# Yasas1994/Jaeger

Measured on AMD Instinct MI355X. Metric: Mbp/s classified (1500bp frags), higher is better.
Workload: dtype f16x3 (split-f16, f32 accumulate)

## Files before the change

### jaeger_amd/csrc/jg_conv_f16_impl.h

```cpp
#include <stdio.h>
#include <stdlib.h>
#include <type_traits>

#include "jg_common.h"

#include "jg_conv_dev.h"

namespace {


#ifdef JG_STAMP
static __device__ unsigned long long jg_stamp_acc[8];
#define JG_ST_DECL unsigned long long st_[8] = {0, 0, 0, 0, 0, 0, 0, 0}; unsigned long long st_t = __builtin_amdgcn_s_memtime(); const unsigned long long st_t0 = st_t
#define JG_ST(idx) do { const unsigned long long n_ = __builtin_amdgcn_s_memtime(); st_[idx] += n_ - st_t; st_t = n_; } while (0)
#define JG_ST_END do { st_[5] = __builtin_amdgcn_s_memtime() - st_t0; if (lane == 0) { for (int q_ = 0; q_ < 8; ++q_) atomicAdd(&jg_stamp_acc[q_], st_[q_]); } } while (0)
#else
#define JG_ST_DECL
#define JG_ST(idx)
#define JG_ST_END
#endif

#ifndef JG_PRIO
#define JG_PRIO 1
#endif
// ... 555 lines not shown
      }
      ++xc;
    }
    JG_ST(3);

    if (a.dbg & 1) {
      if (acc[0][0][0] + acc[1][TN - 1][3] + acc[TM - 1][TN - 1][7] + acc[TM - 1][0][9] == 12345.678f) a.overflow[0] = 2;
    } else if constexpr (JG_FASTEP && TANH && !LUT && CW == 128 && EP != JG_EP_GENERIC && K == 5) {
      JG_PRIO_EPI();
      constexpr bool HAS_ADD = (EP & JG_EP_ADD) != 0;
      constexpr bool HAS_NMD = (EP & (JG_EP_NMD1 | JG_EP_NMD2)) != 0;
      constexpr int N1 = (EP >> 1) & 3, N2 = (EP >> 6) & 3;
      static_assert(N1 != 2 && N2 != 2, "the tanh-GELU builds carry no DyT stage");
      typedef unsigned u32x4 __attribute__((ext_vector_type(4)));
      const Tile &tile = cur[0];
      float vmax = 0.f;
      bool vnan = false;
      const unsigned L4 = 4u * (unsigned)a.L_out;
      unsigned ob[4], om[4], olive = 0;
#pragma unroll
      for (int tm = 0; tm < 4; ++tm) {
        int row, p;
        const bool live = resolve(tile, (wm * 4 + tm) * 32 + i, a.L_out, row, p);
        const int mc = live ? p : 0;
        if constexpr (FLAT) {
          if (!live) row = min(max(row, 0), a.rows - 1);
        }
        ob[tm] = (unsigned)(((row * 8 + 4 * wn) * 4 + h) * a.L_out + mc);
        om[tm] = (unsigned)(row * a.L_out + mc);
        if (live) olive |= 1u << tm;
      }
      struct In {
        u32x4 sh0, sh1, sl0, sl1;
        unsigned char mkb;
      };
      auto fetch = [&](In &q, int b) {
        const int tm = b & 3, tn = b >> 2;
        q.mkb = a.mask_out != nullptr ? a.mask_out[om[tm]] : (unsigned char)1;
        if constexpr (HAS_ADD) {
          if (!(a.dbg & 128)) {
            const unsigned it0 = ob[tm] + (unsigned)(2 * tn) * L4, it1 = it0 + L4;
            q.sh0 = ld_stream(reinterpret_cast<const u32x4 *>(a.addh + it0));
            q.sl0 = ld_stream(reinterpret_cast<const u32x4 *>(a.addh + it0 + 2u * (unsigned)a.L_out));
            q.sh1 = ld_stream(reinterpret_cast<const u32x4 *>(a.addh + it1));
            q.sl1 = ld_stream(reinterpret_cast<const u32x4 *>(a.addh + it1 + 2u * (unsigned)a.L_out));
          } else {
            q.sh0 = q.sh1 = q.sl0 = q.sl1 = u32x4{0u, 0u, 0u, 0u};
          }
        }
      };
      auto swap32 = [](unsigned &lo_half_keeps, unsigned &hi_half_keeps) {
        const auto r = __builtin_amdgcn_permlane32_swap(lo_half_keeps, hi_half_keeps, false, false);
        lo_half_keeps = r[0];
        hi_half_keeps = r[1];
      };
#define JG_DPP(v, ctrl) __uint_as_float((unsigned)__builtin_amdgcn_update_dpp(0, (int)__float_as_uint(v), (ctrl), 0xf, 0xf, false))
      auto lane_reduce = [&](const float (&in)[16], auto op) -> float {
        const bool b2 = (i & 4) != 0, b1 = (i & 2) != 0, b0 = (i & 1) != 0, b3 = (i & 8) != 0;
        float s8[8], s4[4], s2[2];
#pragma unroll
        for (int q = 0; q < 8; ++q) {
          const float keep = b2 ? in[8 + q] : in[q], send = b2 ? in[q] : in[8 + q];
          s8[q] = op(keep, JG_DPP(send, 0x141));
        }
#pragma unroll
        for (int q = 0; q < 4; ++q) {
          const float keep = b1 ? s8[4 + q] : s8[q], send = b1 ? s8[q] : s8[4 + q];
          s4[q] = op(keep, JG_DPP(send, 0x4e));
        }
#pragma unroll
        for (int q = 0; q < 2; ++q) {
          const float keep = b0 ? s4[2 + q] : s4[q], send = b0 ? s4[q] : s4[2 + q];
          s2[q] = op(keep, JG_DPP(send, 0xb1));
        }
        const float keep1 = b3 ? s2[1] : s2[0], send1 = b3 ? s2[0] : s2[1];
        const float v = op(keep1, JG_DPP(send1, 0x128));
        return op(v, __shfl_xor(v, 16, 32));
      };
#undef JG_DPP
      auto reduced_slot = [&](int tn, int &ch) -> size_t {
        const int r = 8 * (int)((i & 4) != 0) + 4 * (int)((i & 2) != 0) + 2 * (int)((i & 1) != 0) + (int)((i & 8) != 0);
        ch = (wn * 2 + tn) * 32 + 8 * (r >> 2) + 4 * h + (r & 3);
        return ((size_t)tile.T * STRIPS + wm) * a.cout + ch;
      };
      f32x2 nmd2[8];
      float pool_acc[16];
      In in0, in1;
      fetch(in0, 0);
      fetch(in1, 1);
      auto do_block = [&](int b, In &q) {
        const int tm = b & 3, tn = b >> 2;
        f32x16 &x = acc[tm][tn];
        const bool live = ((olive >> tm) & 1u) != 0u;
        const float mk = (live && q.mkb != 0) ? 1.f : 0.f;
        const int nb = (wn * 2 + tn) * 32;
        if (tm == 0) {
          if constexpr (HAS_NMD) {
#pragma unroll
            for (int r = 0; r < 8; ++r) nmd2[r] = f32x2{0.f, 0.f};
          }
#pragma unroll
          for (int r = 0; r < 16; ++r) pool_acc[r] = -INFINITY;
        }
        if (!(a.dbg & 32)) {
#pragma unroll
          for (int j = 0; j < 2; ++j) {
            f32x2 v[4];
#pragma unroll
            for (int r = 0; r < 4; ++r) v[r] = f32x2{x[8 * j + 2 * r], x[8 * j + 2 * r + 1]};
            auto st_affine = [&](int row) {
              const float *pr = epiL + (row * 2) * HN + nb + 4 * h + 16 * j;
              const float4 sc0 = *reinterpret_cast<const float4 *>(pr), sc1 = *reinterpret_cast<const float4 *>(pr + 8);
              const float4 of0 = *reinterpret_cast<const float4 *>(pr + HN), of1 = *reinterpret_cast<const float4 *>(pr + HN + 8);
              v[0] = __builtin_elementwise_fma(v[0], f32x2{sc0.x, sc0.y}, f32x2{of0.x, of0.y});
              v[1] = __builtin_elementwise_fma(v[1], f32x2{sc0.z, sc0.w}, f32x2{of0.z, of0.w});
              v[2] = __builtin_elementwise_fma(v[2], f32x2{sc1.x, sc1.y}, f32x2{of1.x, of1.y});
              v[3] = __builtin_elementwise_fma(v[3], f32x2{sc1.z, sc1.w}, f32x2{of1.z, of1.w});
            };
            auto st_add = [&]() {
              const u32x4 qh = j == 0 ? q.sh0 : q.sh1, ql = j == 0 ? q.sl0 : q.sl1;
              unsigned hx = qh[0], hy = qh[1], hz = qh[2], hw_ = qh[3];
              unsigned lx = ql[0], ly = ql[1], lz = ql[2], lw_ = ql[3];
              swap32(hx, hz); swap32(hy, hw_);
              swap32(lx, lz); swap32(ly, lw_);
              v[0] += f32x2{mix_sum<0>(hx, lx), mix_sum<1>(hx, lx)};
              v[1] += f32x2{mix_sum<0>(hy, ly), mix_sum<1>(hy, ly)};
              v[2] += f32x2{mix_sum<0>(hz, lz), mix_sum<1>(hz, lz)};
              v[3] += f32x2{mix_sum<0>(hw_, lw_), mix_sum<1>(hw_, lw_)};
            };
            auto st_gelu = [&]() {
#pragma unroll
              for (int r = 0; r < 4; ++r) v[r] = fast_gelu2(v[r]);
            };
            auto st_nmd = [&]() {
              const f32x2 mk2 = {mk, mk};
#pragma unroll
              for (int r = 0; r < 4; ++r) nmd2[4 * j + r] = __builtin_elementwise_fma(v[r], mk2, nmd2[4 * j + r]);
            };
            st_affine(0);
            if constexpr (EP & JG_EP_NMD1) st_nmd();
            if constexpr (N1 == 1) st_affine(1);
            if constexpr (HAS_ADD) st_add();
            if constexpr (EP & JG_EP_ACT1) st_gelu();
            if constexpr (EP & JG_EP_NMD2) st_nmd();
            if constexpr (N2 == 1) st_affine(N1 ? 2 : 1);
            if constexpr (EP & JG_EP_ACT2) st_gelu();
            if (a.out_f16s) {
              unsigned hp[4], lp[4];
#pragma unroll
              for (int r = 0; r < 4; ++r) {
                typedef _Float16 half2_t __attribute__((ext_vector_type(2)));
                const half2_t hh = {(_Float16)v[r].x, (_Float16)v[r].y};
                hp[r] = *reinterpret_cast<const unsigned *>(&hh);
                const half2_t ll = {(_Float16)mix_rem<0>(v[r].x, hp[r]), (_Float16)mix_rem<1>(v[r].y, hp[r])};
                lp[r] = *reinterpret_cast<const unsigned *>(&ll);
              }
              vmax = fmaxf(fmaxf(vmax, fmaxf(fabsf(v[0].x), fabsf(v[0].y))), fmaxf(fabsf(v[1].x), fabsf(v[1].y)));
              vmax = fmaxf(fmaxf(vmax, fmaxf(fabsf(v[2].x), fabsf(v[2].y))), fmaxf(fabsf(v[3].x), fabsf(v[3].y)));
              vnan = vnan || __builtin_isunordered(v[0].x, v[0].y) || __builtin_isunordered(v[1].x, v[1].y) ||
                     __builtin_isunordered(v[2].x, v[2].y) || __builtin_isunordered(v[3].x, v[3].y);
              swap32(hp[0], hp[2]); swap32(hp[1], hp[3]);
              swap32(lp[0], lp[2]); swap32(lp[1], lp[3]);
              if (live && !(a.dbg & 64)) {
                uint4 *yh = reinterpret_cast<uint4 *>(a.y);
                const unsigned it4 = ob[tm] + (unsigned)(2 * tn + j) * L4;
                const u32x4 vhi = {hp[0], hp[1], hp[2], hp[3]}, vlo = {lp[0], lp[1], lp[2], lp[3]};
                st_stream(vhi, reinterpret_cast<u32x4 *>(yh + it4));
                st_stream(vlo, reinterpret_cast<u32x4 *>(yh + it4 + 2u * (unsigned)a.L_out));
              }
            } else if (a.pool_out != nullptr) {
#pragma unroll
              for (int r = 0; r < 4; ++r) {
                pool_acc[8 * j + 2 * r] = mk != 0.f ? fmaxf(pool_acc[8 * j + 2 * r], v[r].x) : pool_acc[8 * j + 2 * r];
                pool_acc[8 * j + 2 * r + 1] = mk != 0.f ? fmaxf(pool_acc[8 * j + 2 * r + 1], v[r].y) : pool_acc[8 * j + 2 * r + 1];
              }
            } else if (live && !(a.dbg & 64)) {
              float *yf = reinterpret_cast<float *>(a.y) + (size_t)om[tm] * a.cout + nb + 4 * h + 16 * j;
              *reinterpret_cast<float4 *>(yf) = make_float4(v[0].x, v[0].y, v[1].x, v[1].y);
              *reinterpret_cast<float4 *>(yf + 8) = make_float4(v[2].x, v[2].y, v[3].x, v[3].y);
            }
          }
        }
        if (b + 2 < 8) fetch(q, b + 2);
        if (tm == 3) {
          if constexpr (HAS_NMD) {
            float na[16];
#pragma unroll
            for (int r = 0; r < 8; ++r) { na[2 * r] = nmd2[r].x; na[2 * r + 1] = nmd2[r].y; }
            const float rv = lane_reduce(na, [](float x_, float y_) { return x_ + y_; });
            int ch;
            const size_t slot = reduced_slot(tn, ch);
            if (i < 16 && tile.valid) a.nmd_out[slot] = rv;
          }
          if (a.pool_out != nullptr) {
            const float rv = lane_reduce(pool_acc, [](float x_, float y_) { return fmaxf(x_, y_); });
            int ch;
            const size_t slot = reduced_slot(tn, ch);
            if (i < 16 && tile.valid) a.pool_out[slot] = rv;
          }
        }
      };
#pragma unroll
      for (int bp = 0; bp < 4; ++bp) {
        do_block(2 * bp, in0);
        do_block(2 * bp + 1, in1);
      }
      if ((!(vmax <= 65000.0f) || vnan) && a.overflow != nullptr && a.dbg == 0) atomicOr(a.overflow, 1);
      JG_PRIO_MAIN();
    } else {
      JG_PRIO_EPI();
      float vmax = 0.f;
      bool vnan = false;
      float nmd_acc[16];
      float nmd_acc2[16];
      struct Pre {
        uint2 sh[4], sl[4];
        unsigned char mkb;
      };
      auto swap32 = [](unsigned &lo_half_keeps, unsigned &hi_half_keeps) {
        const auto r = __builtin_amdgcn_permlane32_swap(lo_half_keeps, hi_half_keeps, false, false);
        lo_half_keeps = r[0];
        hi_half_keeps = r[1];
      };
      auto item4 = [&](int row, int mc, int nb, int j) -> unsigned {
        const int G = ((nb + ch0) >> 3) + 2 * j + h;
        return (unsigned)(((row * (a.cout_pad >> 4) + (G >> 1)) * 4 + (G & 1)) * a.L_out + mc);
      };
      const bool psplit = GEN && a.psplit != 0;
      const int L_st = psplit ? ((a.L_out + 1) >> 1) : a.L_out;
      auto item4_out = [&](int row, int mc, int nb, int j) -> unsigned {
        if constexpr (GEN) {
          if (psplit) {
            const int G = ((nb + ch0) >> 3) + 2 * j + h, CC = a.cout_pad >> 4;
            return (unsigned)(((row * 2 * CC + (mc & 1) * CC + (G >> 1)) * 4 + (G & 1)) * L_st + (mc >> 1));
          }
        }
        return item4(row, mc, nb, j);
      };
      auto out_pos = [&](const Tile &tile, int tm, int &row, int &mc) -> bool {
        int p;
        bool live = resolve(tile, (wm * TM + tm) * 32 + i, L_res, row, p);
        if constexpr (GEN) {
          if (a.ostride == 2) {
            live = live && !(p & 1);
            p >>= 1;
          }
        }
        mc = live ? p : 0;
        if constexpr (FLAT) {
          if (!live) row = min(max(row, 0), a.rows - 1);
        }
        return live;
      };
      constexpr bool OPOS = !GEN;
      unsigned ob[TM], om[TM], olive = 0;
      size_t o_row = 0, o_mrow = 0;
      unsigned o_step = 0;
      const void *e_y = a.y, *e_addh = a.addh;
      const uint8_t *e_mask = a.mask_out;
      int e_dbg = a.dbg, e_f16s = a.out_f16s;
      float *e_pool = a.pool_out, *e_nmd = a.nmd_out;
      int *e_overflow = a.overflow;
      if constexpr (OPOS) {
        typedef const __attribute__((address_space(4))) ConvHArgs *KArgs;
        KArgs ka = (KArgs)__builtin_amdgcn_kernarg_segment_ptr();
        asm volatile("" : "+s"(ka));
        e_addh = ka->addh;
        e_mask = ka->mask_out;
        e_dbg = ka->dbg;
        e_f16s = ka->out_f16s;
        e_nmd = ka->nmd_out;
        const unsigned Lo = (unsigned)ka->L_out, CC4 = (unsigned)(ka->cout_pad >> 4) * 4u;
        o_step = FLAT ? 2u * Lo : 32u * Lo;
        asm volatile("" : "+s"(o_step));
        if constexpr (!FLAT) {
          o_row = (size_t)cur[0].rowblk * CC4 * Lo * 16u + (size_t)(wn * 8) * o_step;
          o_mrow = (size_t)cur[0].rowblk * Lo;
        }
#pragma unroll
        for (int tm = 0; tm < TM; ++tm) {
          int row, p;
          const bool live = resolve(cur[0], (wm * TM + tm) * 32 + i, (int)Lo, row, p);
          const int mc = live ? p : 0;
          if constexpr (FLAT) {
            if (!live) row = min(max(row, 0), a.rows - 1);
          }
          if (live) olive |= 1u << tm;
          if constexpr (FLAT) {
            om[tm] = (unsigned)row * Lo + (unsigned)mc;
            ob[tm] = ((unsigned)row * CC4 + (unsigned)h) * Lo + (unsigned)mc;
          } else {
            om[tm] = (unsigned)mc;
            ob[tm] = ((unsigned)h * Lo + (unsigned)mc) * 16u;
          }
        }
      }
      auto o_item = [&](const void *base, int tm, int tn, int j, int plane) -> const char * {
        if constexpr (FLAT) {
          return reinterpret_cast<const char *>(base) + ((size_t)(ob[tm] + (unsigned)(((wn * 2 + tn) * 2 + j) * 2 + plane) * o_step) << 4);
        } else {
          return reinterpret_cast<const char *>(base) + (o_row + (size_t)((unsigned)((tn * 2 + j) * 2 + plane) * o_step)) + ob[tm];
        }
      };
      auto o_maskbyte = [&](int tm) -> unsigned char {
        return e_mask != nullptr ? (e_mask + o_mrow)[om[tm]] : (unsigned char)1;
      };
      auto prefetch = [&](Pre &p, const Tile &tile, int tm, int tn) {
        const int nb = (wn * 2 + tn) * 32;
        int orow = 0, mc = 0;
        if constexpr (OPOS) {
          p.mkb = o_maskbyte(tm);
        } else {
          out_pos(tile, tm, orow, mc);
          p.mkb = a.mask_out != nullptr ? a.mask_out[(size_t)orow * a.L_out + mc] : (unsigned char)1;
        }
        if (e_addh != nullptr && !(e_dbg & 128)) {
#pragma unroll
          for (int j = 0; j < 2; ++j) {
            typedef unsigned u32x4 __attribute__((ext_vector_type(4)));
            const u32x4 *src_h, *src_l;
            if constexpr (OPOS) {
              src_h = reinterpret_cast<const u32x4 *>(o_item(e_addh, tm, tn, j, 0));
              src_l = reinterpret_cast<const u32x4 *>(o_item(e_addh, tm, tn, j, 1));
            } else {
              const unsigned it4 = item4(orow, mc, (!GEN || nb + ch0 + 16 * j < a.cout) ? nb : 0, j);
              src_h = reinterpret_cast<const u32x4 *>(a.addh + it4);
              src_l = reinterpret_cast<const u32x4 *>(a.addh + it4 + 2u * (unsigned)a.L_out);
            }
            const u32x4 nh = ld_stream(src_h);
            const u32x4 nl = ld_stream(src_l);
            uint4 vh = make_uint4(nh[0], nh[1], nh[2], nh[3]);
            uint4 vl = make_uint4(nl[0], nl[1], nl[2], nl[3]);
            swap32(vh.x, vh.z); swap32(vh.y, vh.w);
            swap32(vl.x, vl.z); swap32(vl.y, vl.w);
            p.sh[2 * j] = make_uint2(vh.x, vh.y);  p.sh[2 * j + 1] = make_uint2(vh.z, vh.w);
            p.sl[2 * j] = make_uint2(vl.x, vl.y);  p.sl[2 * j + 1] = make_uint2(vl.z, vl.w);
          }
        } else {
#pragma unroll
          for (int g = 0; g < 4; ++g) p.sh[g] = p.sl[g] = make_uint2(0u, 0u);
        }
      };
      auto epi_block = [&](f32x16 &x, const Tile &tile, int tm, int tn) {
        Pre p;
        prefetch(p, tile, tm, tn);
        const int nb = (wn * 2 + tn) * 32;
        bool live;
        if constexpr (OPOS) {
          live = ((olive >> tm) & 1u) != 0u;
        } else {
          int orow_, mc_;
          live = out_pos(tile, tm, orow_, mc_);
        }
        const float mk = p.mkb != 0 ? 1.f : 0.f;
        auto st_affine = [&](int row) {
          const float *pr = epiL + (row * 2) * HN + nb + 4 * h;
#pragma unroll
          for (int g = 0; g < 4; ++g) {
            const float4 sc = *reinterpret_cast<const float4 *>(pr + 8 * g);
            const float4 of = *reinterpret_cast<const float4 *>(pr + HN + 8 * g);
            x[4 * g + 0] = fmaf(x[4 * g + 0], sc.x, of.x);
            x[4 * g + 1] = fmaf(x[4 * g + 1], sc.y, of.y);
            x[4 * g + 2] = fmaf(x[4 * g + 2], sc.z, of.z);
            x[4 * g + 3] = fmaf(x[4 * g + 3], sc.w, of.w);
          }
        };
        auto st_dyt = [&](int row, float alpha, int use_mask) {
          const float *pr = epiL + (row * 2) * HN + nb + 4 * h;
          const float mm = use_mask ? mk : 1.0f;
#pragma unroll
          for (int g = 0; g < 4; ++g) {
            const float4 ga = *reinterpret_cast<const float4 *>(pr + 8 * g);
            const float4 be = *reinterpret_cast<const float4 *>(pr + HN + 8 * g);
            x[4 * g + 0] = (fast_tanh(alpha * x[4 * g + 0]) * ga.x + be.x) * mm;
            x[4 * g + 1] = (fast_tanh(alpha * x[4 * g + 1]) * ga.y + be.y) * mm;
            x[4 * g + 2] = (fast_tanh(alpha * x[4 * g + 2]) * ga.z + be.z) * mm;
            x[4 * g + 3] = (fast_tanh(alpha * x[4 * g + 3]) * ga.w + be.w) * mm;
          }
        };
        auto st_add = [&]() {
#pragma unroll
          for (int g = 0; g < 4; ++g) {
            x[4 * g + 0] += mix_sum<0>(p.sh[g].x, p.sl[g].x);
            x[4 * g + 1] += mix_sum<1>(p.sh[g].x, p.sl[g].x);
            x[4 * g + 2] += mix_sum<0>(p.sh[g].y, p.sl[g].y);
            x[4 * g + 3] += mix_sum<1>(p.sh[g].y, p.sl[g].y);
          }
        };
        auto st_gelu = [&]() {
          constexpr bool TANH_ONLY = TANH || EP == JG_EP_RUNTIME ||
                                     (EP != JG_EP_GENERIC && ((((EP >> 1) & 3) == 2) || (((EP >> 6) & 3) == 2)));
          if (TANH_ONLY || a.act_kind == JG_ACT_GELU_TANH) {
#pragma unroll
            for (int r = 0; r < 16; ++r) x[r] = fast_gelu(x[r]);
          } else if (a.act_kind == JG_ACT_GELU_ERF) {
#pragma unroll
            for (int r = 0; r < 16; ++r) x[r] = gelu_erf(x[r]);
          } else {
#pragma unroll
            for (int r = 0; r < 16; ++r) x[r] = fmaxf(x[r], 0.0f);
          }
        };
        auto st_nmd = [&](int which = 0) {
          const float mkl = live ? mk : 0.f;
          if constexpr (EP == JG_EP_RUNTIME) {
            if (which) {
#pragma unroll
              for (int r = 0; r < 16; ++r) nmd_acc2[r] = fmaf(x[r], mkl, nmd_acc2[r]);
              return;
            }
          }
#pragma unroll
          for (int r = 0; r < 16; ++r) nmd_acc[r] = fmaf(x[r], mkl, nmd_acc[r]);
        };
        if constexpr (EP == JG_EP_GENERIC) {
          for (int q = 0; q < ((e_dbg & 32) ? 0 : a.n_hst); ++q) {
            const HStageArg st = a.hst[q];
            switch (st.kind) {
              case JG_HST_AFFINE: st_affine(st.pad_); break;
              case JG_HST_DYT: st_dyt(st.pad_, st.f0, st.arg); break;
              case JG_HST_ADD: st_add(); break;
              case JG_HST_ACT:
#pragma unroll
                for (int r = 0; r < 16; ++r) x[r] = jg_act(x[r], st.arg);
                break;
              case JG_HST_NMD: st_nmd(); break;
              case JG_HST_MASKMUL:
#pragma unroll
                for (int r = 0; r < 16; ++r) x[r] *= mk;
                break;
              default: break;
            }
          }
        } else if constexpr (EP == JG_EP_RUNTIME) {
          const unsigned e_ = a.ep_rt;
          const int n1 = (int)((e_ >> 1) & 3u), n2 = (int)((e_ >> 6) & 3u);
          st_affine(0);
          if (e_ & JG_EP_NMD1) st_nmd(0);
          if (n1 == 1) st_affine(1);
          else if (n1 == 2) st_dyt(1, a.alpha1, a.dytmask1);
          if (e_ & JG_EP_ADD) st_add();
          if (e_ & JG_EP_ACT1) st_gelu();
          if (e_ & JG_EP_NMD2) st_nmd((e_ & JG_EP_NMD1) ? 1 : 0);
          if (n2 == 1) st_affine(n1 ? 2 : 1);
          else if (n2 == 2) st_dyt(n1 ? 2 : 1, a.alpha2, a.dytmask2);
          if (e_ & JG_EP_ACT2) st_gelu();
        } else if (!(e_dbg & 32)) {
          constexpr int N1 = (EP >> 1) & 3, N2 = (EP >> 6) & 3;
          st_affine(0);
          if constexpr (EP & JG_EP_NMD1) st_nmd();
          if constexpr (N1 == 1) st_affine(1);
          if constexpr (N1 == 2) st_dyt(1, a.alpha1, a.dytmask1);
          if constexpr (EP & JG_EP_ADD) st_add();
          if constexpr (EP & JG_EP_ACT1) st_gelu();
          if constexpr (EP & JG_EP_NMD2) st_nmd();
          if constexpr (N2 == 1) st_affine(N1 ? 2 : 1);
          if constexpr (N2 == 2) st_dyt(N1 ? 2 : 1, a.alpha2, a.dytmask2);
          if constexpr (EP & JG_EP_ACT2) st_gelu();
        }
        if constexpr (GEN) {
          if (psplit) {
#pragma unroll
            for (int r = 0; r < 16; ++r) x[r] *= mk;
          }
        }
        if (e_f16s) {
          uint2 ph[4], pl[4];
#pragma unroll
          for (int g = 0; g < 4; ++g) {
            half4 hh4, ll4;
#pragma unroll
            for (int j = 0; j < 4; ++j) {
              hh4[j] = (_Float16)x[4 * g + j];
              vmax = fmaxf(vmax, fabsf(x[4 * g + j]));
            }
            vnan = vnan || __builtin_isunordered(x[4 * g + 0], x[4 * g + 1]) || __builtin_isunordered(x[4 * g + 2], x[4 * g + 3]);
            ph[g] = *reinterpret_cast<uint2 *>(&hh4);
            ll4[0] = (_Float16)mix_rem<0>(x[4 * g + 0], ph[g].x);
            ll4[1] = (_Float16)mix_rem<1>(x[4 * g + 1], ph[g].x);
            ll4[2] = (_Float16)mix_rem<0>(x[4 * g + 2], ph[g].y);
            ll4[3] = (_Float16)mix_rem<1>(x[4 * g + 3], ph[g].y);
            pl[g] = *reinterpret_cast<uint2 *>(&ll4);
          }
#pragma unroll
          for (int j = 0; j < 2; ++j) {
            unsigned h0 = ph[2 * j].x, h1 = ph[2 * j].y, h2 = ph[2 * j + 1].x, h3 = ph[2 * j + 1].y;
            unsigned l0 = pl[2 * j].x, l1 = pl[2 * j].y, l2 = pl[2 * j + 1].x, l3 = pl[2 * j + 1].y;
            swap32(h0, h2); swap32(h1, h3);
            swap32(l0, l2); swap32(l1, l3);
            x[4 * j + 0] = __uint_as_float(h0); x[4 * j + 1] = __uint_as_float(h1);
            x[4 * j + 2] = __uint_as_float(h2); x[4 * j + 3] = __uint_as_float(h3);
            x[8 + 4 * j + 0] = __uint_as_float(l0); x[8 + 4 * j + 1] = __uint_as_float(l1);
            x[8 + 4 * j + 2] = __uint_as_float(l2); x[8 + 4 * j + 3] = __uint_as_float(l3);
          }
        }
      };
      char *f32_base = nullptr;
      auto store_block = [&](const f32x16 &x, const Tile &tile, int tm, int tn, bool f16s) {
        const int nb = (wn * 2 + tn) * 32;
        if constexpr (OPOS) {
          typedef unsigned u32x4 __attribute__((ext_vector_type(4)));
          if (f16s) {
#pragma unroll
            for (int j = 0; j < 2; ++j) {
              const u32x4 vhi = {__float_as_uint(x[4 * j]), __float_as_uint(x[4 * j + 1]),
                                 __float_as_uint(x[4 * j + 2]), __float_as_uint(x[4 * j + 3])};
              const u32x4 vlo = {__float_as_uint(x[8 + 4 * j]), __float_as_uint(x[8 + 4 * j + 1]),
                                 __float_as_uint(x[8 + 4 * j + 2]), __float_as_uint(x[8 + 4 * j + 3])};
              st_stream(vhi, reinterpret_cast<u32x4 *>(const_cast<char *>(o_item(e_y, tm, tn, j, 0))));
              st_stream(vlo, reinterpret_cast<u32x4 *>(const_cast<char *>(o_item(e_y, tm, tn, j, 1))));
            }
          } else {
            char *yf = f32_base + tn * (32 * 4);
            if constexpr (FLAT) yf += ((size_t)om[tm] * (HN * 4) + 16 * h);
            else yf += om[tm] * (unsigned)(HN * 4) + 16u * (unsigned)h;
#pragma unroll
            for (int g = 0; g < 4; ++g)
              *reinterpret_cast<float4 *>(yf + 32 * g) = make_float4(x[4 * g], x[4 * g + 1], x[4 * g + 2], x[4 * g + 3]);
          }
          return;
        }
        int orow, mc;
        const bool live = out_pos(tile, tm, orow, mc);
        if (live && !(e_dbg & 64)) {
          if (e_f16s) {
            uint4 *yh = reinterpret_cast<uint4 *>(a.y);
#pragma unroll
            for (int j = 0; j < 2; ++j) {
              if (GEN && nb + ch0 + 16 * j >= a.cout) continue;
              const unsigned it4 = item4_out(orow, mc, nb, j);
              typedef unsigned u32x4 __attribute__((ext_vector_type(4)));
              const u32x4 vhi = {__float_as_uint(x[4 * j]), __float_as_uint(x[4 * j + 1]),
                                 __float_as_uint(x[4 * j + 2]), __float_as_uint(x[4 * j + 3])};
              const u32x4 vlo = {__float_as_uint(x[8 + 4 * j]), __float_as_uint(x[8 + 4 * j + 1]),
                                 __float_as_uint(x[8 + 4 * j + 2]), __float_as_uint(x[8 + 4 * j + 3])};
              st_stream(vhi, reinterpret_cast<u32x4 *>(yh + it4));
              st_stream(vlo, reinterpret_cast<u32x4 *>(yh + it4 + 2u * (unsigned)L_st));
              if (GEN && psplit && (a.L_out & 1) && mc == a.L_out - 1) {
                const unsigned itz = it4 + (unsigned)((a.cout_pad >> 4) * 4 * L_st);
                const u32x4 z = {0u, 0u, 0u, 0u};
                st_stream(z, reinterpret_cast<u32x4 *>(yh + itz));
                st_stream(z, reinterpret_cast<u32x4 *>(yh + itz + 2u * (unsigned)L_st));
              }
            }
          } else {
            float *yf = reinterpret_cast<float *>(a.y) + ((size_t)orow * a.L_out + mc) * a.cout + ch0 + nb + 4 * h;
#pragma unroll
            for (int g = 0; g < 4; ++g)
              if (ch0 + nb + 8 * g + 4 * h < a.cout)
                *reinterpret_cast<float4 *>(yf + 8 * g) =
                    make_float4(x[4 * g], x[4 * g + 1], x[4 * g + 2], x[4 * g + 3]);
          }
        }
      };
#define JG_DPP(v, ctrl) __uint_as_float((unsigned)__builtin_amdgcn_update_dpp(0, (int)__float_as_uint(v), (ctrl), 0xf, 0xf, false))
      auto lane_reduce = [&](const float (&in)[16], auto op) -> float {
        const bool b2 = (i & 4) != 0, b1 = (i & 2) != 0, b0 = (i & 1) != 0, b3 = (i & 8) != 0;
        float s8[8], s4[4], s2[2];
#pragma unroll
        for (int q = 0; q < 8; ++q) {
          const float keep = b2 ? in[8 + q] : in[q], send = b2 ? in[q] : in[8 + q];
          s8[q] = op(keep, JG_DPP(send, 0x141));
        }
#pragma unroll
        for (int q = 0; q < 4; ++q) {
          const float keep = b1 ? s8[4 + q] : s8[q], send = b1 ? s8[q] : s8[4 + q];
          s4[q] = op(keep, JG_DPP(send, 0x4e));
        }
#pragma unroll
        for (int q = 0; q < 2; ++q) {
          const float keep = b0 ? s4[2 + q] : s4[q], send = b0 ? s4[q] : s4[2 + q];
          s2[q] = op(keep, JG_DPP(send, 0xb1));
        }
        const float keep1 = b3 ? s2[1] : s2[0], send1 = b3 ? s2[0] : s2[1];
        const float v = op(keep1, JG_DPP(send1, 0x128));
        return op(v, __shfl_xor(v, 16, 32));
      };
      auto reduced_slot = [&](const Tile &tile, int tn, int &ch) -> size_t {
        const int r = 8 * (int)((i & 4) != 0) + 4 * (int)((i & 2) != 0) + 2 * (int)((i & 1) != 0) + (int)((i & 8) != 0);
        ch = ch0 + (wn * 2 + tn) * 32 + 8 * (r >> 2) + 4 * h + (r & 3);
        return ((size_t)tile.T * STRIPS + wm) * a.cout + ch;
      };
      auto nmd_flush = [&](const Tile &tile, int tn) {
        const float v = lane_reduce(nmd_acc, [](float x, float y) { return x + y; });
        int ch;
        const size_t slot = reduced_slot(tile, tn, ch);
        if (i < 16 && tile.valid && ch < a.cout) e_nmd[slot] = v;
      };
      const bool has_nmd = (EP == JG_EP_GENERIC || EP == JG_EP_RUNTIME) ? e_nmd != nullptr : (EP & (JG_EP_NMD1 | JG_EP_NMD2)) != 0;
#pragma unroll
      for (int tn = 0; tn < TN; ++tn) {
#pragma unroll
        for (int r = 0; r < 16; ++r) nmd_acc[r] = 0.f;
        if constexpr (EP == JG_EP_RUNTIME) {
#pragma unroll
          for (int r = 0; r < 16; ++r) nmd_acc2[r] = 0.f;
        }
#pragma unroll
        for (int tm = 0; tm < TM; ++tm) epi_block(acc[tm][tn], cur[0], tm, tn);
        if (has_nmd) nmd_flush(cur[0], tn);
        if constexpr (EP == JG_EP_RUNTIME) {
          if (a.nmd_out2 != nullptr) {
            const float v2 = lane_reduce(nmd_acc2, [](float x, float y) { return x + y; });
            int ch2;
            const size_t slot2 = reduced_slot(cur[0], tn, ch2);
            if (i < 16 && cur[0].valid && ch2 < a.cout) a.nmd_out2[slot2] = v2;
          }
        }
      }
      if constexpr (OPOS) {
        typedef const __attribute__((address_space(4))) ConvHArgs *KArgs;
        KArgs ka = (KArgs)__builtin_amdgcn_kernarg_segment_ptr();
        asm volatile("" : "+s"(ka));
        e_y = ka->y;
        e_pool = ka->pool_out;
        e_overflow = ka->overflow;
      }
      if (e_pool != nullptr) {
        float mkv[TM];
#pragma unroll
        for (int tm = 0; tm < TM; ++tm) {
          bool live;
          unsigned char mb;
          if constexpr (OPOS) {
            live = ((olive >> tm) & 1u) != 0u;
            mb = o_maskbyte(tm);
          } else {
            int orow, mc;
            live = out_pos(cur[0], tm, orow, mc);
            mb = a.mask_out != nullptr ? a.mask_out[(size_t)orow * a.L_out + mc] : (unsigned char)1;
          }
          mkv[tm] = (live && mb != 0) ? 1.f : 0.f;
        }
#pragma unroll
        for (int tn = 0; tn < TN; ++tn) {
          float pa[16];
#pragma unroll
          for (int r = 0; r < 16; ++r) pa[r] = -INFINITY;
#pragma unroll
          for (int tm = 0; tm < TM; ++tm)
#pragma unroll
            for (int r = 0; r < 16; ++r) pa[r] = mkv[tm] != 0.f ? fmaxf(pa[r], acc[tm][tn][r]) : pa[r];
          const float v = lane_reduce(pa, [](float x, float y) { return fmaxf(x, y); });
          int ch;
          const size_t slot = reduced_slot(cur[0], tn, ch);
          if (i < 16 && cur[0].valid && ch < a.cout) e_pool[slot] = v;
        }
      } else if constexpr (OPOS) {
        auto store_tile = [&](bool f16s) {
#pragma unroll
          for (int tm = 0; tm < TM; ++tm) {
            if (!((olive >> tm) & 1u)) continue;
#pragma unroll
            for (int tn = 0; tn < TN; ++tn) store_block(acc[tm][tn], cur[0], tm, tn, f16s);
          }
        };
        if (!(e_dbg & 64)) {
          if (e_f16s) {
            store_tile(true);
          } else {
            f32_base = reinterpret_cast<char *>(const_cast<void *>(e_y)) + (o_mrow * (size_t)HN + (size_t)(wn * 64)) * 4u;
            store_tile(false);
          }
        }
      } else {
#pragma unroll
        for (int tm = 0; tm < TM; ++tm) {
#pragma unroll
          for (int tn = 0; tn < TN; ++tn) store_block(acc[tm][tn], cur[0], tm, tn, false);
        }
      }
      if ((!(vmax <= 65000.0f) || vnan) && e_overflow != nullptr && e_dbg == 0) atomicOr(e_overflow, 1);
      JG_PRIO_MAIN();
    }
    if constexpr (!PIPE) zero_acc();
#pragma unroll
    for (int u = 0; u < NT; ++u) cur[u] = np[u];
    tiles_of(pass + 2, np);
    if constexpr (!LUT) load_bytes(np);
    JG_ST(4);
  }
#ifdef JG_VALU_PROBE
  if (probe[0] + probe[1] + probe[2] + probe[3] + probe[4] + probe[5] + probe[6] + probe[7] == 12345.678f) a.overflow[0] = 4;
#endif
  JG_ST_END;
}

template <int K, unsigned EP, bool FLAT = false, int CW = 128, bool TANH = false, bool PIPE = false>
int launch_ke(jg_engine *e, const ConvHArgs &a, hipStream_t s) {
  const int smem = jg_conv_f16_lds_bytes(K, a.dil);
  static bool attr_set = false;
  if (!attr_set) {
    JG_HIP(hipFuncSetAttribute(reinterpret_cast<const void *>(conv_f16x3_kernel<K, EP, false, FLAT, CW, TANH, PIPE>),
                               hipFuncAttributeMaxDynamicSharedMemorySize, 160 * 1024));
    attr_set = true;
  }
  const int n_tiles = FLAT ? a.flat_tiles : a.rows * a.tiles_m;
  const int n_pairs = (n_tiles + NT - 1) / NT;
  static const bool one_wg = jg_exp_env("JG_ONE_WG") != nullptr;
  int grid = ((smem <= 80 * 1024 && !one_wg) ? 2 : 1) * e->n_cu;
  if (grid > n_pairs) grid = n_pairs;
  ConvHArgs b = a;
  hipLaunchKernelGGL((conv_f16x3_kernel<K, EP, false, FLAT, CW, TANH, PIPE>), dim3((unsigned)grid), dim3(HT), (size_t)smem, s, b);
  JG_HIP(hipGetLastError());
#ifdef JG_STAMP
  {
    unsigned long long h[8], z[8] = {0, 0, 0, 0, 0, 0, 0, 0};
    JG_HIP(hipStreamSynchronize(s));
    JG_HIP(hipMemcpyFromSymbol(h, HIP_SYMBOL(jg_stamp_acc), sizeof(h)));
    JG_HIP(hipMemcpyToSymbol(HIP_SYMBOL(jg_stamp_acc), z, sizeof(z)));
    const double tot = (double)h[5];
    fprintf(stderr, "STAMP k=%d ep=%u rows=%d grid=%d total_cyc/wave=%.0f wait=%.3f barrier=%.3f issue=%.3f lds_mfma=%.3f epilogue=%.3f\n",
            K, EP, a.rows, grid, tot / (grid * 4.0), h[0] / tot, h[1] / tot, h[2] / tot, (h[3] + h[6]) / tot, h[4] / tot);
  }
#endif
  return JG_OK;
}

template <int K, unsigned EP, bool FLAT>
int launch_hot(jg_engine *e, const ConvHArgs &a, hipStream_t s) {
  if constexpr (K == 5) {
#ifdef JG_EXPERIMENT
    if (e->conv_pc == 2 && a.dil == 3 && a.cc_in % 2 == 0 && a.dbg == 0) return launch_ke<5, EP, FLAT, 128, true, true>(e, a, s);
#endif
    return launch_ke<5, EP, FLAT, 128, true>(e, a, s);
  } else {
    return launch_ke<K, EP, FLAT>(e, a, s);
  }
}

#if JG_CONV_PART == 4
template <unsigned EP, int CW, bool TANH = false>
int launch_lut_e(jg_engine *e, const ConvHArgs &a, hipStream_t s) {
  const int smem = jg_conv_lut_lds_bytes(a.k, a.lut_vocab);
  static bool attr_set = false;
  if (!attr_set) {
    JG_HIP(hipFuncSetAttribute(reinterpret_cast<const void *>(conv_f16x3_kernel<0, EP, true, false, CW, TANH>),
                               hipFuncAttributeMaxDynamicSharedMemorySize, 160 * 1024));
    attr_set = true;
  }
  const int n_tiles = a.rows * a.tiles_m;
  constexpr int tper = JG_LUT_WAVES / 2;
  const int n_pairs = (n_tiles + tper - 1) / tper;
  const int grid = a.lut_one_half ? (n_pairs < e->n_cu ? n_pairs : e->n_cu)
                                  : 2 * (n_pairs < e->n_cu / 2 ? n_pairs : e->n_cu / 2);
  hipLaunchKernelGGL((conv_f16x3_kernel<0, EP, true, false, CW, TANH>), dim3((unsigned)grid), dim3(JG_LUT_WAVES * 64), (size_t)smem, s, a);
  JG_HIP(hipGetLastError());
  return JG_OK;
}

int launch_lut(jg_engine *e, const ConvHArgs &a, hipStream_t s) {
  switch (a.ep) {
#define JG_CASE(ep) case (ep): return a.cout == 128 ? launch_lut_e<(ep), 128>(e, a, s) : launch_lut_e<(ep), 129>(e, a, s);
    JG_CASE(0u)
    JG_CASE(JG_EP_NMD1)
    JG_CASE(JG_EP_ACT1)
    JG_CASE(JG_EP_NORM1_AFF | JG_EP_ACT1)
    JG_CASE(JG_EP_NORM1_DYT | JG_EP_ACT1)
    case (JG_EP_NMD1 | JG_EP_NORM1_AFF | JG_EP_ACT1):
      if (a.cout == 128 && a.act_kind == JG_ACT_GELU_TANH) return launch_lut_e<(JG_EP_NMD1 | JG_EP_NORM1_AFF | JG_EP_ACT1), 128, true>(e, a, s);
      return a.cout == 128 ? launch_lut_e<(JG_EP_NMD1 | JG_EP_NORM1_AFF | JG_EP_ACT1), 128>(e, a, s)
                           : launch_lut_e<(JG_EP_NMD1 | JG_EP_NORM1_AFF | JG_EP_ACT1), 129>(e, a, s);
    JG_CASE(JG_EP_NMD1 | JG_EP_NORM1_DYT | JG_EP_ACT1)
    JG_CASE(JG_EP_ACT1 | JG_EP_NORM2_AFF)
    JG_CASE(JG_EP_RUNTIME)
#undef JG_CASE
    default: break;
  }
  jg_set_error("conv lut: stage pattern 0x%x has no compiled epilogue", a.ep);
  return JG_ERR_UNSUPPORTED;
}

#endif

#define JG_ROW_CASES(K)                                                                              \
  switch (a.ep) {                                                                                    \
    case 0u: return launch_ke<K, 0u>(e, a, s);                 \
    case (JG_EP_NMD1): return launch_ke<K, (JG_EP_NMD1)>(e, a, s);                                   \
    case (JG_EP_ACT1):                                    \
      if (K == 5 && a.act_kind == JG_ACT_GELU_TANH) return launch_hot<K, (JG_EP_ACT1), false>(e, a, s); \
      return launch_ke<K, (JG_EP_ACT1)>(e, a, s);                                                     \
    case (JG_EP_NORM1_AFF | JG_EP_ACT1): return launch_ke<K, (JG_EP_NORM1_AFF | JG_EP_ACT1)>(e, a, s); \
    case (JG_EP_NORM1_DYT | JG_EP_ACT1): return launch_ke<K, (JG_EP_NORM1_DYT | JG_EP_ACT1)>(e, a, s); \
    case (JG_EP_ADD | JG_EP_ACT1):                                                                   \
      if (K == 5 && a.act_kind == JG_ACT_GELU_TANH) return launch_hot<K, (JG_EP_ADD | JG_EP_ACT1), false>(e, a, s); \
      return launch_ke<K, (JG_EP_ADD | JG_EP_ACT1)>(e, a, s);                                         \
    case (JG_EP_NORM1_DYT | JG_EP_ADD | JG_EP_ACT1):                                                 \
      return launch_ke<K, (JG_EP_NORM1_DYT | JG_EP_ADD | JG_EP_ACT1)>(e, a, s);                      \
    case (JG_EP_ADD | JG_EP_ACT1 | JG_EP_NMD2 | JG_EP_NORM2_AFF | JG_EP_ACT2):                       \
      if (K == 5 && a.act_kind == JG_ACT_GELU_TANH)                                                  \
        return launch_hot<K, (JG_EP_ADD | JG_EP_ACT1 | JG_EP_NMD2 | JG_EP_NORM2_AFF | JG_EP_ACT2), false>(e, a, s); \
      return launch_ke<K, (JG_EP_ADD | JG_EP_ACT1 | JG_EP_NMD2 | JG_EP_NORM2_AFF | JG_EP_ACT2)>(e, a, s); \
    case (JG_EP_NORM1_DYT | JG_EP_ADD | JG_EP_ACT1 | JG_EP_NMD2 | JG_EP_NORM2_DYT | JG_EP_ACT2):     \
      return launch_ke<K, (JG_EP_NORM1_DYT | JG_EP_ADD | JG_EP_ACT1 | JG_EP_NMD2 | JG_EP_NORM2_DYT | JG_EP_ACT2)>(e, a, s); \
    case (JG_EP_NMD1 | JG_EP_NORM1_AFF | JG_EP_ACT1):                                                \
      return launch_ke<K, (JG_EP_NMD1 | JG_EP_NORM1_AFF | JG_EP_ACT1)>(e, a, s);                     \
    case (JG_EP_NMD1 | JG_EP_NORM1_DYT | JG_EP_ACT1):                                                \
      return launch_ke<K, (JG_EP_NMD1 | JG_EP_NORM1_DYT | JG_EP_ACT1)>(e, a, s);                     \
    case (JG_EP_ADD | JG_EP_ACT1 | JG_EP_NORM2_AFF | JG_EP_ACT2):                                    \
      return launch_ke<K, (JG_EP_ADD | JG_EP_ACT1 | JG_EP_NORM2_AFF | JG_EP_ACT2)>(e, a, s);         \
    case (JG_EP_NORM1_DYT | JG_EP_ADD | JG_EP_ACT1 | JG_EP_NORM2_DYT | JG_EP_ACT2):                  \
      return launch_ke<K, (JG_EP_NORM1_DYT | JG_EP_ADD | JG_EP_ACT1 | JG_EP_NORM2_DYT | JG_EP_ACT2)>(e, a, s); \
    case (JG_EP_ACT1 | JG_EP_NORM2_AFF): return launch_ke<K, (JG_EP_ACT1 | JG_EP_NORM2_AFF)>(e, a, s); \
    case (JG_EP_ACT1 | JG_EP_NORM2_AFF | JG_EP_ACT2):                                                \
      return launch_ke<K, (JG_EP_ACT1 | JG_EP_NORM2_AFF | JG_EP_ACT2)>(e, a, s);                     \
    case (JG_EP_NMD1 | JG_EP_NORM1_AFF | JG_EP_ADD | JG_EP_ACT1):                                    \
      return launch_ke<K, (JG_EP_NMD1 | JG_EP_NORM1_AFF | JG_EP_ADD | JG_EP_ACT1)>(e, a, s);         \
    case (JG_EP_NMD1 | JG_EP_NORM1_AFF | JG_EP_ADD | JG_EP_ACT1 | JG_EP_NORM2_AFF | JG_EP_ACT2):     \
      return launch_ke<K, (JG_EP_NMD1 | JG_EP_NORM1_AFF | JG_EP_ADD | JG_EP_ACT1 | JG_EP_NORM2_AFF | JG_EP_ACT2)>(e, a, s); \
    case (JG_EP_ADD | JG_EP_ACT1 | JG_EP_NMD2):            \
      return launch_ke<K, (JG_EP_ADD | JG_EP_ACT1 | JG_EP_NMD2)>(e, a, s);                           \
    case (JG_EP_NORM1_DYT | JG_EP_ADD | JG_EP_ACT1 | JG_EP_NMD2):                                    \
      return launch_ke<K, (JG_EP_NORM1_DYT | JG_EP_ADD | JG_EP_ACT1 | JG_EP_NMD2)>(e, a, s);         \
    case (JG_EP_NORM1_DYT): return launch_ke<K, (JG_EP_NORM1_DYT)>(e, a, s);                         \
    case (JG_EP_RUNTIME): return launch_ke<K, (JG_EP_RUNTIME)>(e, a, s);                             \
    default: break;                                                                                  \
  }                                                                                                  \
  jg_set_error("conv_f16x3: stage pattern 0x%x has no compiled epilogue", a.ep);                     \
  return JG_ERR_UNSUPPORTED;

}

#if JG_CONV_PART == 1
int jg_conv_f16_part_k5(jg_engine *e, const ConvHArgs &a, hipStream_t s) { JG_ROW_CASES(5) }
#elif JG_CONV_PART == 2
int jg_conv_f16_part_k79(jg_engine *e, const ConvHArgs &a, hipStream_t s) {
  if (a.k == 7) { JG_ROW_CASES(7) }
  { JG_ROW_CASES(9) }
}
#elif JG_CONV_PART == 3
int jg_conv_f16_part_flat(jg_engine *e, const ConvHArgs &a, hipStream_t s) {
  switch (a.ep) {
#define JG_CASE(ep) case (ep): return launch_ke<5, (ep), true>(e, a, s);
#define JG_CASE_HOT(ep)      \
  case (ep):                                                                                                  \
    return a.act_kind == JG_ACT_GELU_TANH ? launch_hot<5, (ep), true>(e, a, s) : launch_ke<5, (ep), true>(e, a, s);
    JG_CASE_HOT(JG_EP_ACT1)
    JG_CASE(JG_EP_NORM1_AFF | JG_EP_ACT1)
    JG_CASE(JG_EP_NORM1_DYT | JG_EP_ACT1)
    JG_CASE_HOT(JG_EP_ADD | JG_EP_ACT1)
    JG_CASE(JG_EP_NORM1_DYT | JG_EP_ADD | JG_EP_ACT1)
    JG_CASE_HOT(JG_EP_ADD | JG_EP_ACT1 | JG_EP_NMD2 | JG_EP_NORM2_AFF | JG_EP_ACT2)
    JG_CASE(JG_EP_NORM1_DYT | JG_EP_ADD | JG_EP_ACT1 | JG_EP_NMD2 | JG_EP_NORM2_DYT | JG_EP_ACT2)
    JG_CASE(JG_EP_ACT1 | JG_EP_NORM2_AFF)
    JG_CASE(JG_EP_ACT1 | JG_EP_NORM2_AFF | JG_EP_ACT2)
    JG_CASE(JG_EP_ADD | JG_EP_ACT1 | JG_EP_NORM2_AFF | JG_EP_ACT2)
    JG_CASE(JG_EP_NORM1_DYT | JG_EP_ADD | JG_EP_ACT1 | JG_EP_NORM2_DYT | JG_EP_ACT2)
    JG_CASE(JG_EP_ADD | JG_EP_ACT1 | JG_EP_NMD2)
    JG_CASE(JG_EP_NORM1_DYT | JG_EP_ADD | JG_EP_ACT1 | JG_EP_NMD2)
    JG_CASE(JG_EP_RUNTIME)
#undef JG_CASE
#undef JG_CASE_HOT
    default: break;
  }
  jg_set_error("conv_f16x3: stage pattern 0x%x has no compiled window-packed epilogue", a.ep);
  return JG_ERR_UNSUPPORTED;
}
#elif JG_CONV_PART == 4
int jg_conv_f16_part_lut(jg_engine *e, const ConvHArgs &a, hipStream_t s) { return launch_lut(e, a, s); }
#elif JG_CONV_PART >= 5 && JG_CONV_PART <= 7
#if JG_CONV_PART == 5
#define JG_NARROW_CW 64
int jg_conv_f16_part_n64(jg_engine *e, const ConvHArgs &a, hipStream_t s) {
#elif JG_CONV_PART == 6
#define JG_NARROW_CW 32
int jg_conv_f16_part_n32(jg_engine *e, const ConvHArgs &a, hipStream_t s) {
#else
#define JG_NARROW_CW 129
int jg_conv_f16_part_g128(jg_engine *e, const ConvHArgs &a, hipStream_t s) {
#endif
  switch (a.ep) {
#define JG_CASE(ep)                                                          \
  case (ep):                                                                 \
    return a.flat ? launch_ke<5, (ep), true, JG_NARROW_CW>(e, a, s) : launch_ke<5, (ep), false, JG_NARROW_CW>(e, a, s);
    JG_CASE(0u)
    JG_CASE(JG_EP_ACT1)
    JG_CASE(JG_EP_NORM1_AFF | JG_EP_ACT1)
    JG_CASE(JG_EP_ADD | JG_EP_ACT1)
    JG_CASE(JG_EP_ADD | JG_EP_ACT1 | JG_EP_NORM2_AFF | JG_EP_ACT2)
    JG_CASE(JG_EP_NMD1 | JG_EP_NORM1_AFF | JG_EP_ACT1)
    JG_CASE(JG_EP_NMD1 | JG_EP_NORM1_AFF | JG_EP_ADD | JG_EP_ACT1)
    JG_CASE(JG_EP_ADD | JG_EP_ACT1 | JG_EP_NMD2 | JG_EP_NORM2_AFF | JG_EP_ACT2)
    JG_CASE(JG_EP_NORM1_DYT | JG_EP_ACT1)
    JG_CASE(JG_EP_NORM1_DYT | JG_EP_ADD | JG_EP_ACT1)
    JG_CASE(JG_EP_NMD1)
    JG_CASE(JG_EP_ADD | JG_EP_ACT1 | JG_EP_NMD2)
    JG_CASE(JG_EP_NORM1_DYT)
    JG_CASE(JG_EP_NORM1_DYT | JG_EP_ADD | JG_EP_ACT1 | JG_EP_NMD2)
    JG_CASE(JG_EP_RUNTIME)
#undef JG_CASE
    default: break;
  }
  jg_set_error("conv_f16x3: stage pattern 0x%x has no compiled narrow-conv epilogue", a.ep);
  return JG_ERR_UNSUPPORTED;
}
#elif JG_CONV_PART >= 8 && JG_CONV_PART <= 13
#define JG_X_CW (((JG_CONV_PART - 8) % 3) == 0 ? 64 : ((JG_CONV_PART - 8) % 3) == 1 ? 32 : 129)
#define JG_X_K ((JG_CONV_PART - 8) / 3 == 0 ? 7 : 9)
#define JG_X_NAME2(p) jg_conv_f16_part_x##p
#define JG_X_NAME(p) JG_X_NAME2(p)
int JG_X_NAME(JG_CONV_PART)(jg_engine *e, const ConvHArgs &a, hipStream_t s) {
  switch (a.ep) {
#define JG_CASE(ep) case (ep): return launch_ke<JG_X_K, (ep), false, JG_X_CW>(e, a, s);
    JG_CASE(0u)
    JG_CASE(JG_EP_ACT1)
    JG_CASE(JG_EP_NORM1_AFF | JG_EP_ACT1)
    JG_CASE(JG_EP_ADD | JG_EP_ACT1)
    JG_CASE(JG_EP_ADD | JG_EP_ACT1 | JG_EP_NORM2_AFF | JG_EP_ACT2)
    JG_CASE(JG_EP_NMD1 | JG_EP_NORM1_AFF | JG_EP_ACT1)
    JG_CASE(JG_EP_NMD1 | JG_EP_NORM1_AFF | JG_EP_ADD | JG_EP_ACT1)
    JG_CASE(JG_EP_ADD | JG_EP_ACT1 | JG_EP_NMD2 | JG_EP_NORM2_AFF | JG_EP_ACT2)
    JG_CASE(JG_EP_NORM1_DYT | JG_EP_ACT1)
    JG_CASE(JG_EP_NORM1_DYT | JG_EP_ADD | JG_EP_ACT1)
    JG_CASE(JG_EP_NMD1)
    JG_CASE(JG_EP_ADD | JG_EP_ACT1 | JG_EP_NMD2)
    JG_CASE(JG_EP_NORM1_DYT)
    JG_CASE(JG_EP_NORM1_DYT | JG_EP_ADD | JG_EP_ACT1 | JG_EP_NMD2)
    JG_CASE(JG_EP_RUNTIME)
#undef JG_CASE
    default: break;
  }
  jg_set_error("conv_f16x3: stage pattern 0x%x has no compiled k = 7 / 9 run-time-geometry epilogue", a.ep);
  return JG_ERR_UNSUPPORTED;
}
#endif
```

Before: 84.59.

## Software-pipeline residual-add loads one block ahead in compiled conv epilogue

For compiled epilogue variants with output positions, the residual-add (addh) loads for the next epilogue block are issued ahead, either at block start or after the first activation, using double-buffered raw registers fenced by sched_barrier. The goal is to hide global load latency behind the current block's math. Mask bytes are also loaded once up front for NMD/DyT variants and reused by the pool path instead of being reloaded. The cost is more live VGPRs for the raw buffers, which could lower occupancy or cause spills, and a more complex variant selection keyed on K, FLAT and TANH.

```diff
diff --git a/jaeger_amd/csrc/jg_conv_f16_impl.h b/jaeger_amd/csrc/jg_conv_f16_impl.h
--- a/jaeger_amd/csrc/jg_conv_f16_impl.h
+++ b/jaeger_amd/csrc/jg_conv_f16_impl.h
@@ -881,14 +881,48 @@
           return reinterpret_cast<const char *>(base) + (o_row + (size_t)((unsigned)((tn * 2 + j) * 2 + plane) * o_step)) + ob[tm];
         }
       };
-      auto o_maskbyte = [&](int tm) -> unsigned char {
-        return e_mask != nullptr ? (e_mask + o_mrow)[om[tm]] : (unsigned char)1;
+      typedef unsigned u32x4 __attribute__((ext_vector_type(4)));
+      struct Raw {
+        u32x4 h0, l0, h1, l1;
+      };
+      constexpr bool COMPILED = EP != JG_EP_GENERIC && EP != JG_EP_RUNTIME;
+      constexpr bool MASK_EARLY = COMPILED && ((EP & (JG_EP_NMD1 | JG_EP_NMD2)) != 0 || ((EP >> 1) & 3) == 2 || ((EP >> 6) & 3) == 2);
+      unsigned char o_mk[TM];
+#pragma unroll
+      for (int tm = 0; tm < TM; ++tm) o_mk[tm] = 1;
+      if constexpr (OPOS && MASK_EARLY) {
+        if (e_mask != nullptr) {
+#pragma unroll
+          for (int tm = 0; tm < TM; ++tm) o_mk[tm] = (e_mask + o_mrow)[om[tm]];
+        }
+      }
+      constexpr bool ADD_CT = COMPILED && (EP & JG_EP_ADD) != 0;
+      const bool o_add = ADD_CT || (e_addh != nullptr && !(e_dbg & 128));
+      constexpr bool HAS_NMD = (EP & (JG_EP_NMD1 | JG_EP_NMD2)) != 0;
+      constexpr bool HAS_DYT = ((EP >> 1) & 3) == 2 || ((EP >> 6) & 3) == 2;
+      constexpr bool AHEAD_FULL = OPOS && ADD_CT && !HAS_NMD && (K != 5 || (!FLAT && (TANH || HAS_DYT)));
+      constexpr bool AHEAD_LATE = OPOS && ADD_CT && !AHEAD_FULL && (K != 5 || !HAS_NMD || TANH || HAS_DYT);
+      auto fetch_add = [&](Raw &q, int tm, int tn) {
+        if (o_add) {
+          q.h0 = ld_stream(reinterpret_cast<const u32x4 *>(o_item(e_addh, tm, tn, 0, 0)));
+          q.l0 = ld_stream(reinterpret_cast<const u32x4 *>(o_item(e_addh, tm, tn, 0, 1)));
+          q.h1 = ld_stream(reinterpret_cast<const u32x4 *>(o_item(e_addh, tm, tn, 1, 0)));
+          q.l1 = ld_stream(reinterpret_cast<const u32x4 *>(o_item(e_addh, tm, tn, 1, 1)));
+        }
+      };
+      auto unswap = [&](Pre &p, int j, const u32x4 &nh, const u32x4 &nl) {
+        uint4 vh = make_uint4(nh[0], nh[1], nh[2], nh[3]);
+        uint4 vl = make_uint4(nl[0], nl[1], nl[2], nl[3]);
+        swap32(vh.x, vh.z); swap32(vh.y, vh.w);
+        swap32(vl.x, vl.z); swap32(vl.y, vl.w);
+        p.sh[2 * j] = make_uint2(vh.x, vh.y);  p.sh[2 * j + 1] = make_uint2(vh.z, vh.w);
+        p.sl[2 * j] = make_uint2(vl.x, vl.y);  p.sl[2 * j + 1] = make_uint2(vl.z, vl.w);
       };
       auto prefetch = [&](Pre &p, const Tile &tile, int tm, int tn) {
         const int nb = (wn * 2 + tn) * 32;
         int orow = 0, mc = 0;
         if constexpr (OPOS) {
-          p.mkb = o_maskbyte(tm);
+          p.mkb = e_mask != nullptr ? (e_mask + o_mrow)[om[tm]] : (unsigned char)1;
         } else {
           out_pos(tile, tm, orow, mc);
           p.mkb = a.mask_out != nullptr ? a.mask_out[(size_t)orow * a.L_out + mc] : (unsigned char)1;
@@ -896,7 +930,6 @@
         if (e_addh != nullptr && !(e_dbg & 128)) {
 #pragma unroll
           for (int j = 0; j < 2; ++j) {
-            typedef unsigned u32x4 __attribute__((ext_vector_type(4)));
             const u32x4 *src_h, *src_l;
             if constexpr (OPOS) {
               src_h = reinterpret_cast<const u32x4 *>(o_item(e_addh, tm, tn, j, 0));
@@ -908,21 +941,17 @@
             }
             const u32x4 nh = ld_stream(src_h);
             const u32x4 nl = ld_stream(src_l);
-            uint4 vh = make_uint4(nh[0], nh[1], nh[2], nh[3]);
-            uint4 vl = make_uint4(nl[0], nl[1], nl[2], nl[3]);
-            swap32(vh.x, vh.z); swap32(vh.y, vh.w);
-            swap32(vl.x, vl.z); swap32(vl.y, vl.w);
-            p.sh[2 * j] = make_uint2(vh.x, vh.y);  p.sh[2 * j + 1] = make_uint2(vh.z, vh.w);
-            p.sl[2 * j] = make_uint2(vl.x, vl.y);  p.sl[2 * j + 1] = make_uint2(vl.z, vl.w);
+            unswap(p, j, nh, nl);
           }
         } else {
 #pragma unroll
           for (int g = 0; g < 4; ++g) p.sh[g] = p.sl[g] = make_uint2(0u, 0u);
         }
       };
-      auto epi_block = [&](f32x16 &x, const Tile &tile, int tm, int tn) {
+      auto epi_block = [&](f32x16 &x, const Tile &tile, int tm, int tn, const Raw &q, auto &&behind_act1) {
         Pre p;
-        prefetch(p, tile, tm, tn);
+        if constexpr (OPOS && COMPILED) p.mkb = o_mk[tm];
+        else prefetch(p, tile, tm, tn);
         const int nb = (wn * 2 + tn) * 32;
         bool live;
         if constexpr (OPOS) {
@@ -958,6 +987,14 @@
           }
         };
         auto st_add = [&]() {
+          if constexpr (OPOS && COMPILED) {
+            if (!o_add) return;
+#ifdef JG_EXPERIMENT
+            if (e_dbg & 128) return;
+#endif
+            unswap(p, 0, q.h0, q.l0);
+            unswap(p, 1, q.h1, q.l1);
+          }
 #pragma unroll
           for (int g = 0; g < 4; ++g) {
             x[4 * g + 0] += mix_sum<0>(p.sh[g].x, p.sl[g].x);
@@ -1032,6 +1069,7 @@
           if constexpr (N1 == 2) st_dyt(1, a.alpha1, a.dytmask1);
           if constexpr (EP & JG_EP_ADD) st_add();
           if constexpr (EP & JG_EP_ACT1) st_gelu();
+          behind_act1();
           if constexpr (EP & JG_EP_NMD2) st_nmd();
           if constexpr (N2 == 1) st_affine(N1 ? 2 : 1);
           if constexpr (N2 == 2) st_dyt(N1 ? 2 : 1, a.alpha2, a.dytmask2);
@@ -1167,6 +1205,8 @@
         if (i < 16 && tile.valid && ch < a.cout) e_nmd[slot] = v;
       };
       const bool has_nmd = (EP == JG_EP_GENERIC || EP == JG_EP_RUNTIME) ? e_nmd != nullptr : (EP & (JG_EP_NMD1 | JG_EP_NMD2)) != 0;
+      Raw raw0, raw1;
+      if constexpr (OPOS && COMPILED) fetch_add(raw0, 0, 0);
 #pragma unroll
       for (int tn = 0; tn < TN; ++tn) {
 #pragma unroll
@@ -1176,7 +1216,19 @@
           for (int r = 0; r < 16; ++r) nmd_acc2[r] = 0.f;
         }
 #pragma unroll
-        for (int tm = 0; tm < TM; ++tm) epi_block(acc[tm][tn], cur[0], tm, tn);
+        for (int tm = 0; tm < TM; ++tm) {
+          const int b = tn * TM + tm;
+          auto ahead = [&]() {
+            if (b + 1 < TM * TN) {
+              __builtin_amdgcn_sched_barrier(0);
+              fetch_add((AHEAD_LATE || (b & 1)) ? raw0 : raw1, (b + 1) % TM, (b + 1) / TM);
+              __builtin_amdgcn_sched_barrier(0);
+            }
+          };
+          if constexpr (AHEAD_FULL) ahead();
+          else if constexpr (OPOS && COMPILED && !AHEAD_LATE) { if (b > 0) fetch_add((b & 1) ? raw1 : raw0, tm, tn); }
+          epi_block(acc[tm][tn], cur[0], tm, tn, (!AHEAD_LATE && (b & 1)) ? raw1 : raw0, [&]() { if constexpr (AHEAD_LATE) ahead(); });
+        }
         if (has_nmd) nmd_flush(cur[0], tn);
         if constexpr (EP == JG_EP_RUNTIME) {
           if (a.nmd_out2 != nullptr) {
@@ -1197,19 +1249,33 @@
       }
       if (e_pool != nullptr) {
         float mkv[TM];
-#pragma unroll
-        for (int tm = 0; tm < TM; ++tm) {
-          bool live;
-          unsigned char mb;
-          if constexpr (OPOS) {
-            live = ((olive >> tm) & 1u) != 0u;
-            mb = o_maskbyte(tm);
-          } else {
-            int orow, mc;
-            live = out_pos(cur[0], tm, orow, mc);
-            mb = a.mask_out != nullptr ? a.mask_out[(size_t)orow * a.L_out + mc] : (unsigned char)1;
-          }
-          mkv[tm] = (live && mb != 0) ? 1.f : 0.f;
+        if constexpr (OPOS && (MASK_EARLY || ADD_CT)) {
+          unsigned char mb[TM];
+#pragma unroll
+          for (int tm = 0; tm < TM; ++tm) mb[tm] = o_mk[tm];
+          if constexpr (!MASK_EARLY) {
+            if (e_mask != nullptr) {
+#pragma unroll
+              for (int tm = 0; tm < TM; ++tm) mb[tm] = (e_mask + o_mrow)[om[tm]];
+            }
+          }
+#pragma unroll
+          for (int tm = 0; tm < TM; ++tm) mkv[tm] = (((olive >> tm) & 1u) != 0u && mb[tm] != 0) ? 1.f : 0.f;
+        } else {
+#pragma unroll
+          for (int tm = 0; tm < TM; ++tm) {
+            bool live;
+            unsigned char mb;
+            if constexpr (OPOS) {
+              live = ((olive >> tm) & 1u) != 0u;
+              mb = e_mask != nullptr ? (e_mask + o_mrow)[om[tm]] : (unsigned char)1;
+            } else {
+              int orow, mc;
+              live = out_pos(cur[0], tm, orow, mc);
+              mb = a.mask_out != nullptr ? a.mask_out[(size_t)orow * a.L_out + mc] : (unsigned char)1;
+            }
+            mkv[tm] = (live && mb != 0) ? 1.f : 0.f;
+          }
         }
 #pragma unroll
         for (int tn = 0; tn < TN; ++tn) {
```

After: 85.37 (median of 6 runs). About the same (+0.9%).
